# madmann91/bvh

Measured on AMD Instinct MI355X. Metric: Mrays/s closest-hit (1M-tri scene), higher is better.
Workload: dtype f32; 1 GPU; soup_1m: 1,000,000-triangle random soup (M3), worst-case incoherent; robust traversal, DefaultBuilder with thread pool (mini-trees) Quality::High built on the GPU (the reference's default configuration is thread pool + High); rays reordered for coherence inside the timed pass (library default for this tree size); tris=1000000, nodes=1866439, ray_batches=4, parallelism=single GPU, launched_by=single process

## Files before the change

### bvh_amd/csrc/ray_key.h

```cpp
#pragma once

namespace bvh_amd {

namespace {

__device__ inline float rcp_fast(float x) { return __builtin_amdgcn_rcpf(x); }
__device__ inline double rcp_fast(double x) { return 1.0 / x; }
template <typename T>
__device__ inline uint32_t ray_key(const T (&r)[8], T lx, T ly, T lz, T sx, T sy, T sz, uint32_t cells, int hilbert_bits, int class_bits, T class_scale) {
    const T q[3] = { (r[0] - lx) * sx, (r[1] - ly) * sy, (r[2] - lz) * sz };
    uint32_t code = 0;
    uint32_t cell[3];
#pragma unroll
    for (int k = 0; k < 3; ++k) {
        T v = q[k];
        v = v > T(0) ? v : T(0);
        cell[k] = v >= T(cells - 1) ? cells - 1 : static_cast<uint32_t>(v);
    }
    if (hilbert_bits > 0) {
        uint32_t X[3] = { cell[2], cell[1], cell[0] };
        const uint32_t M = 1u << (hilbert_bits - 1);
        for (uint32_t Q = M; Q > 1; Q >>= 1) {
            const uint32_t P = Q - 1;
#pragma unroll
            for (int a = 0; a < 3; ++a) {
                if (X[a] & Q) X[0] ^= P;
                else { const uint32_t t = (X[0] ^ X[a]) & P; X[0] ^= t; X[a] ^= t; }
            }
        }
        X[1] ^= X[0]; X[2] ^= X[1];
        uint32_t t = 0;
        for (uint32_t Q = M; Q > 1; Q >>= 1) if (X[2] & Q) t ^= Q - 1;
        X[0] ^= t; X[1] ^= t; X[2] ^= t;
        cell[2] = X[0]; cell[1] = X[1]; cell[0] = X[2];
    }
#pragma unroll
    for (int k = 0; k < 3; ++k) {
        const uint32_t c = cell[k];
        uint32_t s = (c & 1u) | ((c & 2u) << 2) | ((c & 4u) << 4) | ((c & 8u) << 6) | ((c & 16u) << 8) | ((c & 32u) << 10) | ((c & 64u) << 12) | ((c & 128u) << 14);
        code |= s << k;
    }
    const uint32_t oct = (Num<T>::sign(r[3]) ? 1u : 0u) | (Num<T>::sign(r[4]) ? 2u : 0u) | (Num<T>::sign(r[5]) ? 4u : 0u);
    if (class_bits > 0) {
        const T l[3] = { lx, ly, lz }, sc[3] = { sx, sy, sz };
        T t0 = r[6], t1 = r[7], d2 = T(0), diag2 = T(0);
#pragma unroll
        for (int k = 0; k < 3; ++k) {
            const T ext = sc[k] > T(0) ? T(cells) * rcp_fast(sc[k]) : T(0);
            const T inv = rcp_fast(r[3 + k]);
            const T a = (l[k] - r[k]) * inv, b = (l[k] + ext - r[k]) * inv;
            const T lo_t = a < b ? a : b, hi_t = a < b ? b : a;
            t0 = lo_t > t0 ? lo_t : t0; t1 = hi_t < t1 ? hi_t : t1;
            d2 += r[3 + k] * r[3 + k]; diag2 += ext * ext;
        }
        const uint32_t top = (1u << class_bits) - 1u;
        uint32_t cls = 0;
        const T len = t1 > t0 ? t1 - t0 : T(0);
        if (class_bits == 1) cls = len * len * d2 * class_scale * class_scale >= diag2 && diag2 > T(0) ? 1u : 0u;
        else {
            const T rel = diag2 > T(0) ? len * Num<T>::sqrt_(d2) / Num<T>::sqrt_(diag2) * class_scale : T(0);
            cls = rel >= T(top) ? top : rel > T(0) ? static_cast<uint32_t>(rel) : 0u;
        }
        cls = top - cls;
        const int code_bits = 3 * (hilbert_bits > 0 ? hilbert_bits : 31 - __clz(cells));
        const uint32_t high = code >> (code_bits - 3), low = (code & ((1u << (code_bits - 3)) - 1u)) >> class_bits;
        code = (((high << class_bits) | cls) << (code_bits - 3 - class_bits)) | low;
    }
    return (code << 3) | oct;
}

}

}
```

### bvh_amd/csrc/trace_body.inc

```
#ifndef BVH_TRACE_COOP
#define BVH_TRACE_COOP false
#endif
    constexpr int kDepth = kLdsDepth;
    constexpr int kSpill = 64 - kDepth;
    __shared__ uint32_t lds_stack[kDepth * kBlock];
    uint32_t spill[kSpill];
    const int tid = threadIdx.x;
    const int lane = tid & (kWave - 1);
    const uint64_t lanes_below = (uint64_t{1} << lane) - 1;

    bool have = false, done = false, drained = false, nan_ray = false;
    uint32_t part = a.parts > 1 ? blockIdx.x % a.parts : 0, parts_left = a.parts;
    unsigned long long ray_id = 0;
    T org[3], dir[3], inv[3], aux[3];
    T tmin = 0, tmax = 0;
    uint32_t oct[3] = {0, 0, 0};
    uint32_t top = 0, sp = 0;
    uint32_t hit_prim = BVH_AMD_INVALID;
    T hit_t = 0, hit_u = 0, hit_v = 0;
    unsigned long long n_pairs = 0, n_tests = 0, n_leaves = 0;
#if defined(BVH_AMD_DEVELOPER) && defined(__HIPCC__)
    unsigned long long wt_begin = 0, wt_last_refill = 0, wt_rays = 0, wt_refill_ticks = 0, wt_refills = 0;
    if (a.wave_times) wt_begin = __builtin_amdgcn_s_memrealtime();
#endif

    auto deep_slot = [&](uint32_t i) { return a.deep + (size_t{blockIdx.x} * kBlock + tid) * a.deep_cap + i; };
    auto push = [&](uint32_t v) {
        if (sp < kDepth) lds_stack[sp * kBlock + tid] = v;
        else if (!Deep) spill[min(sp - kDepth, static_cast<uint32_t>(kSpill - 1))] = v;
        else if (sp < kDepth + kSpill) spill[sp - kDepth] = v;
        else *deep_slot(min(sp - (kDepth + kSpill), a.deep_cap - 1)) = v;
        ++sp;
    };
    auto pop = [&]() -> uint32_t {
        --sp;
        uint32_t v = lds_word(&lds_stack[min(sp, static_cast<uint32_t>(kDepth - 1)) * kBlock + tid]);
        if (sp >= kDepth) {
            if (!Deep) v = spill[min(sp - kDepth, static_cast<uint32_t>(kSpill - 1))];
            else if (sp < kDepth + kSpill) v = spill[sp - kDepth];
            else v = *deep_slot(min(sp - (kDepth + kSpill), a.deep_cap - 1));
        }
        return v;
    };

    for (;;) {
        const uint64_t idle = __ballot(!have);
        const int n_idle = __popcll(idle);
        if (!drained && (n_idle >= a.refill_threshold || n_idle == kWave)) {
#if defined(BVH_AMD_DEVELOPER) && defined(__HIPCC__)
            unsigned long long wt_t0 = 0;
            if (a.wave_times) wt_t0 = __builtin_amdgcn_s_memrealtime();
#endif
            unsigned long long base = 0, part_end = a.n;
            if (a.one_shot) {
                base = (static_cast<unsigned long long>(blockIdx.x) * (kBlock / kWave) + (tid >> 6)) * kWave;
                drained = true;
            } else {
                if (lane == 0) base = atomicAdd(a.work + part * kTicketStride, static_cast<unsigned long long>(n_idle));
                base = __shfl(base, 0) + part * a.part_size;
                part_end = min(a.n, (part + 1ull) * a.part_size);
                if (base + n_idle >= part_end) {
                    part = part + 1 == a.parts ? 0 : part + 1;
                    if (--parts_left == 0) drained = true;
                } else if (a.stagger && part_end - (base + n_idle) < static_cast<unsigned long long>(a.stagger) * ((blockIdx.x * 8u) / gridDim.x)) {
                    drained = true;
                }
            }
            if (!have) {
                const unsigned long long ticket = base + __popcll(idle & lanes_below);
                if (ticket < part_end) {
                    const bool once = (a.stream_hints & 1u) != 0;
                    const unsigned long long my = a.order ? (once ? load_word_nt(a.order + ticket) : a.order[ticket]) : ticket;
                    T r[8];
                    if (D == 3) { if (once) load_ray_nt(a.rays + 8 * my, r); else load_ray(a.rays + 8 * my, r); }
                    else {
                        T q[6];
                        load_ray2(a.rays + 6 * my, q);
                        r[0] = q[0]; r[1] = q[1]; r[2] = T(0); r[3] = q[2]; r[4] = q[3]; r[5] = T(0); r[6] = q[4]; r[7] = q[5];
                    }
#pragma unroll
                    for (int k = 0; k < D; ++k) { org[k] = r[k]; dir[k] = r[3 + k]; }
                    ray_constants<T, Robust, D>(org, dir, inv, aux, oct);
                    tmin = r[6]; tmax = r[7];
                    nan_ray = !(tmin == tmin) || !(tmax == tmax);
                    ray_id = my;
                    have = true; done = false;
                    sp = 0;
                    top = a.root_index;
                    hit_prim = BVH_AMD_INVALID; hit_t = tmax; hit_u = 0; hit_v = 0;
                }
            }
#if defined(BVH_AMD_DEVELOPER) && defined(__HIPCC__)
            if (a.wave_times) {
                asm volatile("s_waitcnt vmcnt(0)" ::: "memory");
                wt_last_refill = __builtin_amdgcn_s_memrealtime(); wt_rays += __popcll(__ballot(have)) - (kWave - n_idle);
                wt_refill_ticks += wt_last_refill - wt_t0; ++wt_refills;
            }
#endif
        }
        if (__ballot(have) == 0) {
            if (drained) break;
            continue;
        }

        for (;;) {
            const bool inner = have && !done && (top & kCountMask) == 0;
            const uint64_t inner_mask = __ballot(inner);
            if (!inner_mask) break;
            const int parked = __popcll(__ballot(have && !done && (top & kCountMask) != 0));
            if (parked >= a.leaf_threshold) break;
            T lb[6], rb[6];
            uint32_t li = 0, ri = 0;
            if constexpr (BVH_TRACE_COOP) coop_load_pair(a.pairs, a.pair_bytes, inner ? (top >> (kCountBits + 1)) : 0xFFFFFFFFu, lane, lb, rb, li, ri);
            if (inner) {
                if constexpr (!BVH_TRACE_COOP) load_pair(a.pairs + (top >> (kCountBits + 1)), lb, rb, li, ri);
                if (Stats) ++n_pairs;
                T l0, l1, r0, r1;
                slab_pair<T, Robust, D>(lb, rb, org, inv, aux, oct, tmin, tmax, l0, l1, r0, r1);
                const bool hl = !nan_ray && l0 <= l1, hr = !nan_ray && r0 <= r1;
                if (hl) {
                    uint32_t near_i = li;
                    if (hr) {
                        uint32_t far_i = ri;
                        if (!Any && l0 > r0) { near_i = ri; far_i = li; }
                        push(far_i);
                    }
                    top = near_i;
                } else if (hr) {
                    top = ri;
                } else if (sp == 0) {
                    done = true;
                } else {
                    top = pop();
                }
            }
        }

        if (have && !done && (top & kCountMask) != 0) {
            const uint32_t first = top >> kCountBits, count = top & kCountMask;
            if (Stats) ++n_leaves;
            for (uint32_t i = first; i < first + count; ++i) {
                if (Stats) ++n_tests;
                if (Leaf == LEAF_TRIANGLE) {
// ... 66 lines not shown
```

### bvh_amd/csrc/trace_device.h

```cpp
#pragma once

#if defined(__HIPCC__)
#define BVH_AMD_KEEP_APART(v) asm volatile("" : "+v"(v))
#else
#define BVH_AMD_KEEP_APART(v) asm volatile("" : "+r"(v))
#endif

namespace bvh_amd {

namespace {

constexpr int kBlock = 256;
constexpr int kLdsDepth = 20;
constexpr int kRefillThreshold = 36;
constexpr int kRefillThresholdSmall = 20;
constexpr int kLeafThreshold = 12;
constexpr int kCoopRefillAny = 20, kCoopLeafAny = 20;
constexpr int kCoopRefillHeavy = 12, kCoopLeafHeavy = 12;


template <typename T> struct Num;
template <> struct Num<float> {
    static constexpr float kMax = 3.402823466e+38f, kEps = 1.1920928955078125e-07f;
    __device__ static bool finite(float x) { return (__float_as_uint(x) & 0x7F800000u) != 0x7F800000u; }
// ... 17 lines not shown
    __device__ static double sqrt_(double x) { return __builtin_sqrt(x); }
    __device__ static double abs_(double x) { return __builtin_fabs(x); }
    __device__ static double copysign_(double a, double b) { return __builtin_copysign(a, b); }
    __device__ static double max_num(double a, double b) { return __builtin_fmax(a, b); }
    __device__ static double min_num(double a, double b) { return __builtin_fmin(a, b); }
};

template <typename T> __device__ inline T pick_min(T a, T b) { return a < b ? a : b; }
template <typename T> __device__ inline T pick_max(T a, T b) { return a > b ? a : b; }

template <typename T> __device__ inline T dot3(T a0, T a1, T a2, T b0, T b1, T b2) {
    return ((T(0) + a0 * b0) + a1 * b1) + a2 * b2;
}
__device__ inline uint32_t lds_word(const uint32_t* shared) {
#if defined(__HIP_DEVICE_COMPILE__)
    typedef __attribute__((address_space(3))) const volatile uint32_t LdsWord;
    return *(LdsWord*)shared;
#else
    return *shared;
#endif
}

template <typename T> __device__ inline T dot2(T a0, T a1, T b0, T b1) { return (T(0) + a0 * b0) + a1 * b1; }

template <typename T, bool Robust, int D>
__device__ inline void ray_constants(const T (&org)[3], const T (&dir)[3], T (&inv)[3], T (&aux)[3], uint32_t (&oct)[3]) {
#pragma unroll
    for (int k = 0; k < D; ++k) {
        const T d = dir[k];
        const T iv = Robust ? T(1) / d : (Num<T>::abs_(d) <= Num<T>::kEps ? Num<T>::copysign_(Num<T>::kMax, d) : T(1) / d);
        inv[k] = iv;
        aux[k] = Robust ? (Num<T>::finite(iv) ? Num<T>::bump2(iv) : iv) : (-iv) * org[k];
        oct[k] = Num<T>::sign(d) ? 1u : 0u;
    }
}

template <typename T, bool Robust, int D>
__device__ inline void slab_pair(const T (&lb)[6], const T (&rb)[6], const T (&org)[3], const T (&inv)[3], const T (&aux)[3], const uint32_t (&oct)[3],
                                 T tmin, T tmax, T& l0, T& l1, T& r0, T& r1) {
    l0 = tmin; l1 = tmax; r0 = tmin; r1 = tmax;
#pragma unroll
    for (int k = 0; k < D; ++k) {
        const T ln = oct[k] ? lb[2 * k + 1] : lb[2 * k], lf = oct[k] ? lb[2 * k] : lb[2 * k + 1];
        const T rn = oct[k] ? rb[2 * k + 1] : rb[2 * k], rf = oct[k] ? rb[2 * k] : rb[2 * k + 1];
        T la, lz, ra, rz;
        if (Robust) {
            la = (ln - org[k]) * inv[k]; lz = (lf - org[k]) * aux[k];
            ra = (rn - org[k]) * inv[k]; rz = (rf - org[k]) * aux[k];
        } else {
            la = Num<T>::fma_(ln, inv[k], aux[k]); lz = Num<T>::fma_(lf, inv[k], aux[k]);
            ra = Num<T>::fma_(rn, inv[k], aux[k]); rz = Num<T>::fma_(rf, inv[k], aux[k]);
        }
        l0 = Num<T>::max_num(la, l0); l1 = Num<T>::min_num(lz, l1);
        r0 = Num<T>::max_num(ra, r0); r1 = Num<T>::min_num(rz, r1);
    }
}

constexpr uint32_t kTicketStride = 16;

template <typename T>
struct TraceArgs {
    const PairNode<T>* pairs;
    const T* prims;
    const T* rays;
    typename HitOf<T>::Type* hits;
    unsigned long long n;
    unsigned long long* work;
    unsigned long long part_size;
    uint32_t parts;
    bvh_amd_counters* counters;
    const uint32_t* order;
    uint32_t* deep;
    uint32_t deep_cap;
    uint32_t root_index;
    int refill_threshold;
    int leaf_threshold;
    uint32_t coop;
    uint32_t prim_stride;
    uint32_t stream_hints;
    uint32_t stagger;
    uint32_t one_shot;
    unsigned long long* wave_times;
    uint32_t pair_bytes = 0;
};

__device__ inline void load_pair(const PairNode<float>* p, float (&lb)[6], float (&rb)[6], uint32_t& li, uint32_t& ri) {
    const float4* q = reinterpret_cast<const float4*>(p);
    float4 a = q[0], b = q[1], c = q[2];
    uint2 d = reinterpret_cast<const uint2*>(p)[6];
    lb[0] = a.x; lb[1] = a.y; lb[2] = a.z; lb[3] = a.w; lb[4] = b.x; lb[5] = b.y;
    rb[0] = b.z; rb[1] = b.w; rb[2] = c.x; rb[3] = c.y; rb[4] = c.z; rb[5] = c.w;
    li = d.x; ri = d.y;
}
__device__ inline void load_pair(const PairNode<double>* p, double (&lb)[6], double (&rb)[6], uint32_t& li, uint32_t& ri) {
    const double2* q = reinterpret_cast<const double2*>(p);
#pragma unroll
    for (int i = 0; i < 3; ++i) { double2 v = q[i]; lb[2 * i] = v.x; lb[2 * i + 1] = v.y; }
#pragma unroll
    for (int i = 0; i < 3; ++i) { double2 v = q[3 + i]; rb[2 * i] = v.x; rb[2 * i + 1] = v.y; }
    uint2 d = reinterpret_cast<const uint2*>(p)[12];
    li = d.x; ri = d.y;
}

#if defined(__HIPCC__)
template <int CTRL> __device__ inline uint32_t quad_perm(uint32_t v) {
    return static_cast<uint32_t>(__builtin_amdgcn_mov_dpp(static_cast<int>(v), CTRL, 0xF, 0xF, true));
}
template <bool ByTwo> __device__ inline void quad_exchange4(uint32_t (&a)[4], uint32_t (&b)[4]) {
    const uint64_t lower = ByTwo ? 0x3333333333333333ull : 0x5555555555555555ull;
    uint32_t n0, n1, n2, n3;
    if (ByTwo)
        asm("s_nop 1\n\ts_mov_b64 vcc, %12\n\t"
            "v_cndmask_b32_dpp %0, %4, %8, vcc quad_perm:[2,3,0,1] row_mask:0xf bank_mask:0xf\n\t"
            "v_cndmask_b32_dpp %1, %5, %9, vcc quad_perm:[2,3,0,1] row_mask:0xf bank_mask:0xf\n\t"
            "v_cndmask_b32_dpp %2, %6, %10, vcc quad_perm:[2,3,0,1] row_mask:0xf bank_mask:0xf\n\t"
            "v_cndmask_b32_dpp %3, %7, %11, vcc quad_perm:[2,3,0,1] row_mask:0xf bank_mask:0xf\n\t"
            "s_not_b64 vcc, vcc\n\t"
            "v_cndmask_b32_dpp %4, %8, %4, vcc quad_perm:[2,3,0,1] row_mask:0xf bank_mask:0xf\n\t"
            "v_cndmask_b32_dpp %5, %9, %5, vcc quad_perm:[2,3,0,1] row_mask:0xf bank_mask:0xf\n\t"
            "v_cndmask_b32_dpp %6, %10, %6, vcc quad_perm:[2,3,0,1] row_mask:0xf bank_mask:0xf\n\t"
            "v_cndmask_b32_dpp %7, %11, %7, vcc quad_perm:[2,3,0,1] row_mask:0xf bank_mask:0xf"
            : "=&v"(n0), "=&v"(n1), "=&v"(n2), "=&v"(n3), "+v"(b[0]), "+v"(b[1]), "+v"(b[2]), "+v"(b[3])
            : "v"(a[0]), "v"(a[1]), "v"(a[2]), "v"(a[3]), "s"(lower) : "vcc", "scc");
    else
        asm("s_nop 1\n\ts_mov_b64 vcc, %12\n\t"
            "v_cndmask_b32_dpp %0, %4, %8, vcc quad_perm:[1,0,3,2] row_mask:0xf bank_mask:0xf\n\t"
            "v_cndmask_b32_dpp %1, %5, %9, vcc quad_perm:[1,0,3,2] row_mask:0xf bank_mask:0xf\n\t"
            "v_cndmask_b32_dpp %2, %6, %10, vcc quad_perm:[1,0,3,2] row_mask:0xf bank_mask:0xf\n\t"
            "v_cndmask_b32_dpp %3, %7, %11, vcc quad_perm:[1,0,3,2] row_mask:0xf bank_mask:0xf\n\t"
            "s_not_b64 vcc, vcc\n\t"
            "v_cndmask_b32_dpp %4, %8, %4, vcc quad_perm:[1,0,3,2] row_mask:0xf bank_mask:0xf\n\t"
            "v_cndmask_b32_dpp %5, %9, %5, vcc quad_perm:[1,0,3,2] row_mask:0xf bank_mask:0xf\n\t"
            "v_cndmask_b32_dpp %6, %10, %6, vcc quad_perm:[1,0,3,2] row_mask:0xf bank_mask:0xf\n\t"
            "v_cndmask_b32_dpp %7, %11, %7, vcc quad_perm:[1,0,3,2] row_mask:0xf bank_mask:0xf"
            : "=&v"(n0), "=&v"(n1), "=&v"(n2), "=&v"(n3), "+v"(b[0]), "+v"(b[1]), "+v"(b[2]), "+v"(b[3])
            : "v"(a[0]), "v"(a[1]), "v"(a[2]), "v"(a[3]), "s"(lower) : "vcc", "scc");
    a[0] = n0; a[1] = n1; a[2] = n2; a[3] = n3;
}
#elif defined(BVH_HOST_WAVE64)
template <int CTRL> inline uint32_t quad_perm(uint32_t v) {
    const int l = static_cast<int>(threadIdx.x) & 63;
    return wave_read(v, (l & ~3) | ((CTRL >> (2 * (l & 3))) & 3), true);
}
template <bool ByTwo> inline void quad_exchange4(uint32_t (&a)[4], uint32_t (&b)[4]) {
    const int l = static_cast<int>(threadIdx.x) & 63, bit = ByTwo ? 2 : 1, partner = l ^ bit;
    const bool lower = (l & bit) == 0;
    for (int i = 0; i < 4; ++i) {
        const uint32_t pa = wave_read(a[i], partner, true), pb = wave_read(b[i], partner, true);
        const uint32_t na = lower ? a[i] : pb, nb = lower ? pa : b[i];
        a[i] = na; b[i] = nb;
    }
}
#endif
constexpr uint32_t kNoRecordAt = 0xFFFFFFFFu << 6;
#if defined(__HIPCC__)
using PairRsrc = __amdgpu_buffer_rsrc_t;
__device__ inline PairRsrc pair_rsrc(const void* base, uint32_t bytes) {
    return __builtin_amdgcn_make_buffer_rsrc(const_cast<void*>(base), 0, static_cast<int>(bytes), 0x00020000);
}
__device__ inline uint4 load_chunk(PairRsrc r, uint32_t at) {
    const auto v = __builtin_amdgcn_raw_buffer_load_b128(r, static_cast<int>(at), 0, 0);
    return uint4{v[0], v[1], v[2], v[3]};
}
#elif defined(BVH_HOST_WAVE64)
struct PairRsrc { const char* base; };
inline PairRsrc pair_rsrc(const void* base, uint32_t) { return PairRsrc{static_cast<const char*>(base)}; }
// ... 130 lines not shown
```

### bvh_amd/csrc/traverse.hip

```cpp

#include "common.h"
#include "trace_device.h"
#include "ray_key.h"

#include <algorithm>
#include <cstdlib>
#include <mutex>
#include <thread>
#include <type_traits>
#include <vector>

namespace bvh_amd {

namespace {

thread_local const char* g_last_kernel = "";
thread_local bool g_last_reordered = false;
thread_local int g_last_query_launches = 0;
thread_local int g_last_plan[4] = {0, 0, 0, 0};

struct KernelTimer {
    static constexpr size_t kRing = 256;
    bool on = false;
    size_t count = 0;
    std::pair<hipEvent_t, hipEvent_t> ring[kRing] = {};
    hipEvent_t begin[kRing] = {};
    bool begin_armed = false;
};
KernelTimer& kernel_timer() { static thread_local KernelTimer t; return t; }

template <typename T, bool Any, bool Robust, int Leaf, bool Stats, int D = 3, bool Deep = false>
__global__ void __launch_bounds__(kBlock) trace_kernel(TraceArgs<T> a) {
#include "trace_body.inc"
}

template <typename T, bool Any, bool Robust, int Leaf, bool Stats>
__global__ void __launch_bounds__(kBlock, 8) trace_kernel_coop(TraceArgs<T> a) {
    constexpr int D = 3;
    constexpr bool Deep = false;
#undef BVH_TRACE_COOP
#define BVH_TRACE_COOP true
#include "trace_body.inc"
#undef BVH_TRACE_COOP
}

template <typename T, bool Any, bool Robust, int Leaf, bool Stats, int D>
__global__ void __launch_bounds__(kBlock, sizeof(T) == 4 ? 8 : 4) trace_kernel_coop_nd(TraceArgs<T> a) {
    constexpr bool Deep = false;
#undef BVH_TRACE_COOP
#define BVH_TRACE_COOP true
#include "trace_body.inc"
#undef BVH_TRACE_COOP
}

template <typename T, bool Any, bool Robust, int Leaf>
__global__ void __launch_bounds__(kBlock) trace_kernel_plan_search(TraceArgs<T> a) {
    constexpr int D = 3;
    constexpr bool Deep = false, Stats = false;
#include "trace_body.inc"
}
template <typename T, bool Any, bool Robust, int Leaf>
__global__ void __launch_bounds__(kBlock, 8) trace_kernel_coop_plan_search(TraceArgs<T> a) {
    constexpr int D = 3;
    constexpr bool Deep = false, Stats = false;
#undef BVH_TRACE_COOP
#define BVH_TRACE_COOP true
#include "trace_body.inc"
#undef BVH_TRACE_COOP
}

#if defined(BVH_AMD_DEVELOPER)
__global__ void __launch_bounds__(256) k_check_order(const uint32_t* order, uint32_t n, uint32_t* bad) {
    const uint32_t i = blockIdx.x * 256 + threadIdx.x;
    if (i < n && order[i] >= n) {
        const uint32_t k = atomicAdd(&bad[0], 1u);
        if (k < 3) { bad[1 + 2 * k] = i; bad[2 + 2 * k] = order[i]; }
    }
}
#endif

template <typename T>
__global__ void __launch_bounds__(1024) ray_keys_kernel(const T* rays, uint32_t n, T lx, T ly, T lz, T sx, T sy, T sz, uint32_t* keys, uint32_t cells,
                                                        int hilbert_bits, int class_bits, T class_scale, uint32_t* hist, uint32_t tiles) {
    __shared__ uint32_t h[256];
    if (threadIdx.x < 256) h[threadIdx.x] = 0;
    __syncthreads();
    const uint32_t base = blockIdx.x * uint32_t(kRadixTileU32);
#pragma unroll
    for (int s0 = 0; s0 < kRadixTileU32 / 1024; ++s0) {
        const uint32_t i = base + uint32_t(s0) * 1024u + threadIdx.x;
        if (i < n) {
            T r[8];
            load_ray_nt(rays + 8ull * i, r);
            const uint32_t key = ray_key<T>(r, lx, ly, lz, sx, sy, sz, cells, hilbert_bits, class_bits, class_scale);
            keys[i] = key;
            atomicAdd(&h[key & 0xFFu], 1u);
        }
    }
    __syncthreads();
    if (threadIdx.x < 256) hist[size_t{threadIdx.x} * tiles + blockIdx.x] = h[threadIdx.x];
}

__global__ void __launch_bounds__(256) ray_entry_keys_kernel(const float* rays, uint32_t n, const PairNode<float>* pairs, uint32_t root_index, int depth,
                                                             uint32_t* keys) {
    const uint32_t i = blockIdx.x * 256 + threadIdx.x;
    if (i >= n) return;
    float r[8];
    load_ray(rays + 8ull * i, r);
    const float inv[3] = { 1.0f / r[3], 1.0f / r[4], 1.0f / r[5] };
    uint32_t cur = root_index, path = 0;
    int level = 0;
    for (; level < depth && (cur & kCountMask) == 0; ++level) {
        float lb[6], rb[6];
        uint32_t li, ri;
        load_pair(pairs + (cur >> (kCountBits + 1)), lb, rb, li, ri);
        float t0[2] = { r[6], r[6] }, t1[2] = { r[7], r[7] };
#pragma unroll
        for (int k = 0; k < 3; ++k) {
            const float a0 = (lb[2 * k] - r[k]) * inv[k], a1 = (lb[2 * k + 1] - r[k]) * inv[k];
            const float b0 = (rb[2 * k] - r[k]) * inv[k], b1 = (rb[2 * k + 1] - r[k]) * inv[k];
            t0[0] = fmaxf(t0[0], fminf(a0, a1)); t1[0] = fminf(t1[0], fmaxf(a0, a1));
            t0[1] = fmaxf(t0[1], fminf(b0, b1)); t1[1] = fminf(t1[1], fmaxf(b0, b1));
        }
        const bool hl = t0[0] <= t1[0], hr = t0[1] <= t1[1];
        if (!hl && !hr) break;
        const bool right = hl && hr ? t0[1] < t0[0] : hr;
        path = (path << 1) | (right ? 1u : 0u);
        cur = right ? ri : li;
    }
    path <<= (depth - level);
    const uint32_t oct = (Num<float>::sign(r[3]) ? 1u : 0u) | (Num<float>::sign(r[4]) ? 2u : 0u) | (Num<float>::sign(r[5]) ? 4u : 0u);
    keys[i] = (path << 3) | oct;
}

template <typename H>
__global__ void __launch_bounds__(256) original_ids_kernel(H* hits, size_t n, const uint32_t* prim_ids, uint32_t prim_count) {
    const size_t i = blockIdx.x * size_t{256} + threadIdx.x;
    if (i >= n) return;
    const uint32_t p = hits[i].prim;
    if (p < prim_count) hits[i].prim = prim_ids[p];
}

thread_local int t_refill = -1, t_leaf = -1, t_coop = -1, t_parts = -1;
struct Experiments { int grid_blocks = -1, stream_hints = -1, tri_stride = -1, key_curve = -1, key_bits = -1, wave_times = -1, one_shot = -1,
                     key_class_bits = -1, key_class_scale = -1, stagger = -1; };
constexpr int kKeyClassBits = 0, kKeyClassScalePercent = 500;
constexpr uint32_t kStaggerHeavy = 100000, kStaggerLight = 50000, kStaggerDouble = 20000;
thread_local bool g_last_classes = false;
thread_local float g_search_ns[5] = {0, 0, 0, 0, 0};
thread_local int g_search_count[5] = {0, 0, 0, 0, 0};
thread_local unsigned g_search_dropped = 0;
thread_local Experiments t_exp;
#if defined(BVH_AMD_DEVELOPER)
constexpr size_t kWaveTimeWords = 6, kWaveTimeWaves = 8 * 256 * (kBlock / kWave) * 2;
thread_local unsigned long long* t_wave_times = nullptr;
thread_local size_t t_wave_times_waves = 0;
#endif
thread_local std::pair<hipEvent_t, hipEvent_t>* t_calibration = nullptr;

int coop_fetch_forced() {
    static const int knob = BVH_DEV_INT("BVH_AMD_COOP", -1);
    return t_coop >= 0 ? (t_coop != 0) : knob < 0 ? -1 : (knob != 0);
}

struct Grid { int blocks = 0; };

template <typename K>
int persistent_grid(K kernel, int device, Grid& g) {
    int per_cu = 0, cus = 0;
    BVH_HIP_TRY(hipOccupancyMaxActiveBlocksPerMultiprocessor(&per_cu, kernel, kBlock, 0), BVH_AMD_ERR_HIP);
    BVH_HIP_TRY(hipDeviceGetAttribute(&cus, hipDeviceAttributeMultiprocessorCount, device), BVH_AMD_ERR_HIP);
    if (per_cu < 1) per_cu = 1;
    if (per_cu > 8) per_cu = 8;
    g.blocks = per_cu * cus;
    return BVH_AMD_OK;
}

template <typename T, bool Any, bool Robust, int Leaf, bool Stats, int D, bool Deep, bool Coop = false>
int launch_variant_d(const BvhImpl<T>& b, const TraceArgs<T>& args, hipStream_t stream, const char* name) {
    static thread_local int cached_blocks[16] = {0};
    void (*kernel)(TraceArgs<T>) = nullptr;
    constexpr bool CoopNd = Coop && !(std::is_same_v<T, float> && D == 3);
    if constexpr (CoopNd) kernel = trace_kernel_coop_nd<T, Any, Robust, Leaf, Stats, D>;
    else if constexpr (Coop) kernel = trace_kernel_coop<T, Any, Robust, Leaf, Stats>;
    else kernel = trace_kernel<T, Any, Robust, Leaf, Stats, D, Deep>;
    if constexpr (std::is_same_v<T, float> && D == 3 && !Deep && !Stats) {
        if (t_calibration) {
            if constexpr (Coop) kernel = trace_kernel_coop_plan_search<T, Any, Robust, Leaf>;
            else kernel = trace_kernel_plan_search<T, Any, Robust, Leaf>;
        }
    }
    int& blocks = cached_blocks[b.device & 15];
    if (blocks == 0) {
        Grid g;
        int rc = persistent_grid(kernel, b.device, g);
        if (rc) return rc;
        blocks = g.blocks;
    }
    unsigned long long need = (args.n + kBlock - 1) / kBlock;
    int grid = static_cast<int>(need < static_cast<unsigned long long>(blocks) ? need : blocks);
    if (args.one_shot) grid = static_cast<int>(need);
    else if constexpr (!Coop && std::is_same_v<T, float>) {
        int cus = blocks / 7 > 0 ? blocks / 7 : 1;
        (void)hipDeviceGetAttribute(&cus, hipDeviceAttributeMultiprocessorCount, b.device);
        const int cap = 6 * cus;
        if (grid > cap) grid = cap;
    }
    static const int grid_env = BVH_DEV_INT("BVH_AMD_GRID_BLOCKS", 0);
    if (!args.one_shot) {
        if (grid_env > 0 && grid > grid_env) grid = grid_env;
        if (t_exp.grid_blocks > 0 && grid > t_exp.grid_blocks) grid = t_exp.grid_blocks;
    }
    if (grid < 1) grid = 1;
    (void)name;
    static const std::string head = std::string(CoopNd ? "trace_kernel_coop_nd<" : Coop ? "trace_kernel_coop<" : "trace_kernel<") + (std::is_same_v<T, float> ? "float" : "double") + ", " +
                                    (Any ? "true" : "false") + ", " + (Robust ? "true" : "false") + ", " + std::to_string(Leaf) + ", " + (Stats ? "true" : "false");
    static const std::string symbol = CoopNd ? head + ", " + std::to_string(D) + ">" : Coop ? head + ">" : head + ", " + std::to_string(D) + ", " + (Deep ? "true" : "false") + ">";
    g_last_kernel = symbol.c_str();
    KernelTimer& timer = kernel_timer();
    hipEvent_t stop = nullptr;
    if (timer.on) {
        std::pair<hipEvent_t, hipEvent_t>& ev = timer.ring[timer.count % KernelTimer::kRing];
        if (!timer.begin_armed && timer.begin[timer.count % KernelTimer::kRing]) {
            (void)hipEventDestroy(timer.begin[timer.count % KernelTimer::kRing]);
            timer.begin[timer.count % KernelTimer::kRing] = nullptr;
        }
        timer.begin_armed = false;
        if (!ev.first) {
            BVH_HIP_TRY(hipEventCreate(&ev.first), BVH_AMD_ERR_HIP);
            BVH_HIP_TRY(hipEventCreate(&ev.second), BVH_AMD_ERR_HIP);
        }
        BVH_HIP_TRY(hipEventRecord(ev.first, stream), BVH_AMD_ERR_HIP);
        stop = ev.second;
        ++timer.count;
    }
    if (t_calibration) (void)hipEventRecord(t_calibration->first, stream);
#if defined(BVH_AMD_DEVELOPER)
    TraceArgs<T> timed_args = args;
    if (t_exp.wave_times > 0 && size_t(grid) * (kBlock / kWave) <= kWaveTimeWaves) {
        if (!t_wave_times) BVH_HIP_TRY(hipMalloc(&t_wave_times, kWaveTimeWaves * kWaveTimeWords * sizeof(unsigned long long)), BVH_AMD_ERR_HIP);
        t_wave_times_waves = size_t(grid) * (kBlock / kWave);
        BVH_HIP_TRY(hipMemsetAsync(t_wave_times, 0, t_wave_times_waves * kWaveTimeWords * sizeof(unsigned long long), stream), BVH_AMD_ERR_HIP);
        timed_args.wave_times = t_wave_times;
    }
    hipLaunchKernelGGL(kernel, dim3(grid), dim3(kBlock), 0, stream, timed_args);
#else
    hipLaunchKernelGGL(kernel, dim3(grid), dim3(kBlock), 0, stream, args);
#endif
    BVH_HIP_TRY(hipGetLastError(), BVH_AMD_ERR_HIP);
    if (t_calibration) (void)hipEventRecord(t_calibration->second, stream);
    if (stop) BVH_HIP_TRY(hipEventRecord(stop, stream), BVH_AMD_ERR_HIP);
    return BVH_AMD_OK;
}

template <typename T, bool Any, bool Robust, int Leaf, bool Stats, int D>
int launch_variant(const BvhImpl<T>& b, const TraceArgs<T>& args, hipStream_t stream, const char* name) {
    if (args.deep) return launch_variant_d<T, Any, Robust, Leaf, Stats, D, true>(b, args, stream, name);
    if (args.coop && b.pair_count < (size_t{1} << (std::is_same_v<T, float> ? 26 : 25))) return launch_variant_d<T, Any, Robust, Leaf, Stats, D, false, true>(b, args, stream, name);
    return launch_variant_d<T, Any, Robust, Leaf, Stats, D, false>(b, args, stream, name);
}

#define BVH_VARIANT(T, ANY, ROB, LEAF, STATS) \
    launch_variant<T, ANY, ROB, LEAF, STATS, D>(b, args, stream, D == 3 ? "trace_kernel<" #T "," #ANY "," #ROB "," #LEAF "," #STATS ">" \
                                                                        : "trace_kernel<" #T "," #ANY "," #ROB "," #LEAF "," #STATS ",2>")

template <typename T, int Leaf, int D = 3>
int dispatch(const BvhImpl<T>& b, const TraceArgs<T>& args, unsigned flags, bool stats, hipStream_t stream) {
    const bool any = flags & BVH_AMD_RAY_ANY_HIT, rob = flags & BVH_AMD_RAY_ROBUST;
    if (stats) {
        if (any) return rob ? BVH_VARIANT(T, true, true, Leaf, true) : BVH_VARIANT(T, true, false, Leaf, true);
        return rob ? BVH_VARIANT(T, false, true, Leaf, true) : BVH_VARIANT(T, false, false, Leaf, true);
    }
    if (any) return rob ? BVH_VARIANT(T, true, true, Leaf, false) : BVH_VARIANT(T, true, false, Leaf, false);
    return rob ? BVH_VARIANT(T, false, true, Leaf, false) : BVH_VARIANT(T, false, false, Leaf, false);
}

}

void last_launch_plan(int out[4]) { for (int k = 0; k < 4; ++k) out[k] = g_last_plan[k]; }
void set_tuning(int refill, int leaf, int coop, int parts) { t_refill = refill; t_leaf = leaf; t_coop = coop; t_parts = parts; }
int set_experiment(const char* name, int value) {
    const std::string k = name ? name : "";
    if (k == "grid_blocks") t_exp.grid_blocks = value;
    else if (k == "stream_hints") t_exp.stream_hints = value;
    else if (k == "tri_stride") t_exp.tri_stride = value;
    else if (k == "key_curve") t_exp.key_curve = value;
    else if (k == "key_bits") t_exp.key_bits = value;
    else if (k == "step_events") set_step_events(value);
    else if (k == "one_shot") t_exp.one_shot = value;
    else if (k == "stagger") t_exp.stagger = value;
    else if (k == "key_class_bits") t_exp.key_class_bits = value;
    else if (k == "key_class_scale") t_exp.key_class_scale = value;
    else if (k == "wave_times") {
#if defined(BVH_AMD_DEVELOPER)
        t_exp.wave_times = value;
#else
        return fail(BVH_AMD_ERR_ARG, "bvh_amd_experiment: 'wave_times' exists in the developer library only (python -m bvh_amd.build --developer)");
#endif
    }
    else if (k == "reset") { t_exp = Experiments{}; set_step_events(-1); }
    else return fail(BVH_AMD_ERR_ARG, "bvh_amd_experiment: unknown knob '" + k + "'");
    return BVH_AMD_OK;
}
int wave_times(unsigned long long* out, size_t capacity_waves, size_t* n_waves) {
#if defined(BVH_AMD_DEVELOPER)
    if (n_waves) *n_waves = t_wave_times_waves;
    if (!out || !t_wave_times) return BVH_AMD_OK;
    BVH_HIP_TRY(hipDeviceSynchronize(), BVH_AMD_ERR_HIP);
    BVH_HIP_TRY(hipMemcpy(out, t_wave_times, std::min(capacity_waves, t_wave_times_waves) * kWaveTimeWords * sizeof(unsigned long long), hipMemcpyDeviceToHost), BVH_AMD_ERR_HIP);
    return BVH_AMD_OK;
#else
    (void)out; (void)capacity_waves;
    if (n_waves) *n_waves = 0;
    return fail(BVH_AMD_ERR_ARG, "bvh_amd_wave_times: developer library only");
#endif
}
void last_plan_search(float ns_per_ray[5], int measurements[5], unsigned* dropped) {
    for (int c = 0; c < 5; ++c) { if (ns_per_ray) ns_per_ray[c] = g_search_ns[c]; if (measurements) measurements[c] = g_search_count[c]; }
    if (dropped) *dropped = g_search_dropped;
}
const char* last_kernel_name() { return g_last_kernel; }
bool last_launch_reordered() { return g_last_reordered; }
int last_query_launches() { return g_last_query_launches; }
void set_last_query_launches(int launches) { g_last_query_launches = launches; }

void kernel_timing(bool on) {
    KernelTimer& t = kernel_timer();
    t.on = on;
    t.count = 0;
}

int kernel_times(float* ms_out, size_t capacity, size_t* count_out) {
    KernelTimer& t = kernel_timer();
    const size_t have = std::min<size_t>(t.count, KernelTimer::kRing), n = std::min(have, capacity);
    for (size_t i = 0; i < n; ++i) {
        const std::pair<hipEvent_t, hipEvent_t>& ev = t.ring[(t.count - n + i) % KernelTimer::kRing];
        BVH_HIP_TRY(hipEventSynchronize(ev.second), BVH_AMD_ERR_HIP);
        BVH_HIP_TRY(hipEventElapsedTime(&ms_out[i], ev.first, ev.second), BVH_AMD_ERR_HIP);
    }
    if (count_out) *count_out = n;
    return BVH_AMD_OK;
}

int reorder_times(float* ms_out, size_t capacity, size_t* count_out) {
    KernelTimer& t = kernel_timer();
    const size_t have = std::min<size_t>(t.count, KernelTimer::kRing), n = std::min(have, capacity);
    for (size_t i = 0; i < n; ++i) {
        const size_t k = (t.count - n + i) % KernelTimer::kRing;
        ms_out[i] = 0.0f;
        if (!t.begin[k]) continue;
        BVH_HIP_TRY(hipEventSynchronize(t.ring[k].first), BVH_AMD_ERR_HIP);
        BVH_HIP_TRY(hipEventElapsedTime(&ms_out[i], t.begin[k], t.ring[k].first), BVH_AMD_ERR_HIP);
    }
    if (count_out) *count_out = n;
    return BVH_AMD_OK;
}

template <typename T>
static int to_original_ids(const BvhImpl<T>& b, typename HitOf<T>::Type* d_hits, size_t n, hipStream_t stream) {
    if (!b.d_prim_ids) return fail(BVH_AMD_ERR_ARG, "intersect_rays: BVH has no device prim ids");
    hipLaunchKernelGGL(original_ids_kernel<typename HitOf<T>::Type>, dim3(static_cast<unsigned>((n + 255) / 256)), dim3(256), 0, stream, d_hits, n,
                       b.d_prim_ids, static_cast<uint32_t>(b.prim_count));
    BVH_HIP_TRY(hipGetLastError(), BVH_AMD_ERR_HIP);
    return BVH_AMD_OK;
}

constexpr float kReorderMinVisits = 100.0f;

struct Plan { bool reorder; bool coop; int refill, leaf; bool classes = false; };

template <typename T>
static int launch_planned(const BvhImpl<T>& b, int leaf_kind, const T* d_prims, const T* d_rays, size_t n, unsigned flags,
                          typename HitOf<T>::Type* d_hits, bvh_amd_counters* d_counters, hipStream_t stream, const Plan* plan)
{
    if (n == 0) return BVH_AMD_OK;
// ... 29 lines not shown
        if (ev) timer.begin_armed = hipEventRecord(ev, stream) == hipSuccess;
    }
    TraceArgs<T> args{};
    args.pairs = b.d_pairs; args.prims = d_prims; args.rays = d_rays; args.hits = d_hits;
    args.pair_bytes = static_cast<uint32_t>(std::min<size_t>(b.pair_count * sizeof(PairNode<T>), 0xFFFFFFFFu));
    args.n = n; args.work = work; args.counters = d_counters; args.root_index = b.root_index;
    args.order = nullptr;
    args.prim_stride = leaf_kind == LEAF_TRIANGLE ? (t_exp.tri_stride > 0 ? static_cast<uint32_t>(t_exp.tri_stride) : 12u) : 4u;
    args.stream_hints = 0;
    args.one_shot = (t_exp.one_shot >= 0 ? t_exp.one_shot > 0 : n <= (size_t{1} << 18)) && !d_counters ? 1u : 0u;
    static const int parts_env = BVH_DEV_INT("BVH_AMD_PARTS", 0);
    args.parts = t_parts > 0 ? std::min(t_parts, 256) : parts_env > 0 ? std::min(parts_env, 256) : n < 65536 ? 1 : 8;
    args.part_size = ((n + args.parts - 1) / args.parts + 63) / 64 * 64;
    args.deep = nullptr; args.deep_cap = 0;
    StreamScope scope(stream);
    void* deep_mem = nullptr;
    void* sort_mem = nullptr;
    ScratchTag deep_tag, sort_tag;
    auto release = [&](int rc) {
        (void)hipEventRecord(slot_event, stream);
        { std::lock_guard<std::mutex> lock(b.work_mutex); b.work_busy[slot] = false; }
        if (deep_mem) scratch_free(deep_mem, deep_tag);
        if (sort_mem) scratch_free(sort_mem, sort_tag);
        return rc;
    };
    if (d_counters) {
        const hipError_t e = hipMemsetAsync(d_counters, 0, sizeof(bvh_amd_counters), stream);
        if (e != hipSuccess) return release(fail(BVH_AMD_ERR_HIP, std::string("intersect_rays: hipMemsetAsync: ") + hipGetErrorString(e)));
    }
    {
        int rc = tree_depth<T>(b, stream);
        if (rc) return release(rc);
        const int max_depth = b.max_depth.load();
        if (max_depth > 64) {
            int cus = 0;
            if (hipDeviceGetAttribute(&cus, hipDeviceAttributeMultiprocessorCount, b.device) != hipSuccess) return release(fail(BVH_AMD_ERR_HIP, "intersect_rays: hipDeviceGetAttribute"));
            const size_t lanes = size_t{8} * cus * kBlock;
            const size_t cap = static_cast<size_t>(max_depth - 64 + 1);
            if (lanes * cap > (size_t{1} << 32))
                return release(fail(BVH_AMD_ERR_UNSUPPORTED, "intersect_rays: the tree is too deep for the traversal stack (" + std::to_string(max_depth) + " levels)"));
            const hipError_t e = scratch_alloc(&deep_mem, lanes * cap * sizeof(uint32_t), &deep_tag);
            if (e != hipSuccess) { deep_mem = nullptr; return release(fail(BVH_AMD_ERR_HIP, std::string("intersect_rays: stack spill buffer: ") + hipGetErrorString(e))); }
            args.deep = static_cast<uint32_t*>(deep_mem); args.deep_cap = static_cast<uint32_t>(cap);
            args.one_shot = 0;
        }
    }
    static const int refill_env = BVH_DEV_INT("BVH_AMD_REFILL", 0);
    static const int leaf_env = BVH_DEV_INT("BVH_AMD_LEAF", 0);
    const bool beyond_l2 = b.pair_count * sizeof(PairNode<T>) > (size_t{32} << 20);
    const bool heavy = beyond_l2 && b.expected_visits.load() >= kReorderMinVisits;
    const bool any_hit = (flags & BVH_AMD_RAY_ANY_HIT) != 0;
    const int forced = coop_fetch_forced();
    const bool coop_capable = true;
    if (plan) {
        args.coop = coop_capable && plan->coop ? 1u : 0u;
        args.refill_threshold = plan->refill; args.leaf_threshold = plan->leaf;
    } else {
        args.coop = (coop_capable && (forced >= 0 ? forced != 0 : (any_hit || (heavy && n >= (size_t{1} << 21))))) ? 1u : 0u;
        const int refill_lane = n <= (size_t{1} << 21) && std::is_same_v<T, float> ? kRefillThresholdSmall : kRefillThreshold;
        const int refill_default = !args.coop ? refill_lane : any_hit ? kCoopRefillAny : heavy ? kCoopRefillHeavy : kCoopRefillAny;
        const int leaf_default = !args.coop ? kLeafThreshold : any_hit ? kCoopLeafAny : heavy ? kCoopLeafHeavy : kCoopLeafAny;
        args.refill_threshold = t_refill > 0 ? t_refill : refill_env > 0 ? refill_env : refill_default;
        args.leaf_threshold = t_leaf > 0 ? t_leaf : leaf_env > 0 ? leaf_env : leaf_default;
    }
    auto zero_tickets = [&]() -> int {
        const hipError_t e = hipMemsetAsync(work, 0, size_t{args.parts} * kTicketStride * sizeof(unsigned long long), stream);
        return e == hipSuccess ? BVH_AMD_OK : fail(BVH_AMD_ERR_HIP, std::string("intersect_rays: hipMemsetAsync: ") + hipGetErrorString(e));
    };
    if (b.dim == 2) {
        if (leaf_kind != LEAF_SPHERE) return release(fail(BVH_AMD_ERR_ARG, "intersect_rays: a 2D BVH traces circles (Sphere<T, 2>) only"));
        if (const int rc0 = zero_tickets()) return release(rc0);
        int rc2 = dispatch<T, LEAF_SPHERE, 2>(b, args, flags, d_counters != nullptr, stream);
        if (rc2 == BVH_AMD_OK && (flags & BVH_AMD_RAY_ORIGINAL_IDS)) rc2 = to_original_ids<T>(b, d_hits, n, stream);
        return release(rc2);
    }
    const bool reorder = (flags & BVH_AMD_RAY_SORTED) ? n > 4096
                       : (flags & BVH_AMD_RAY_UNSORTED) ? false
                       : plan ? plan->reorder && n > 4096
                       : n >= (size_t{1} << 20) && beyond_l2 && b.expected_visits.load() >= kReorderMinVisits;
    g_last_reordered = reorder && n < (size_t{1} << 31);
    args.stream_hints = t_exp.stream_hints >= 0 ? static_cast<uint32_t>(t_exp.stream_hints) : g_last_reordered ? 1u : 0u;
    args.parts = t_parts > 0 ? std::min(t_parts, 256) : parts_env > 0 ? std::min(parts_env, 256) : n < 65536 ? 1 : g_last_reordered ? 8 : 32;
    args.part_size = ((n + args.parts - 1) / args.parts + 63) / 64 * 64;
    if (const int rc0 = zero_tickets()) return release(rc0);
    if (g_last_reordered) {
        const uint32_t n32 = static_cast<uint32_t>(n);
        const size_t words = 4 * n + radix_sort_hist_words(n32, 1);
        hipError_t e = scratch_alloc(&sort_mem, words * sizeof(uint32_t), &sort_tag);
        if (e != hipSuccess) {
            sort_mem = nullptr;
            (void)hipGetLastError();
            if (flags & BVH_AMD_RAY_SORTED) return release(fail(BVH_AMD_ERR_HIP, std::string("intersect_rays: no scratch for BVH_AMD_RAY_SORTED: ") + hipGetErrorString(e)));
            g_last_reordered = false;
        }
    }
    if (g_last_reordered) {
        const uint32_t n32 = static_cast<uint32_t>(n);
        uint32_t *keys = static_cast<uint32_t*>(sort_mem), *vals = keys + n, *kt = vals + n, *vt = kt + n, *hist = vt + n;
        T lo[3], sc[3];
        if (const int rc0 = b.wait_refit()) return release(rc0);
        for (int k = 0; k < 3; ++k) {
            const T ext = b.root_bounds[2 * k + 1] - b.root_bounds[2 * k];
            lo[k] = b.root_bounds[2 * k];
            sc[k] = ext > T(0) ? T(64) / ext : T(0);
        }
        static const int entry_depth = std::min(29, BVH_DEV_INT("BVH_AMD_RAY_KEY_DEPTH", 0));
        int key_bits = 21;
        bool entry_keys = false, first_hist_done = false;
        if constexpr (std::is_same_v<T, float>) entry_keys = entry_depth > 0 && b.dim == 3;
        if constexpr (std::is_same_v<T, float>) {
            if (entry_keys) {
                hipLaunchKernelGGL(ray_entry_keys_kernel, dim3((n32 + 255) / 256), dim3(256), 0, stream, d_rays, n32, args.pairs, args.root_index, entry_depth, keys);
                key_bits = entry_depth + 3;
            }
        }
        if (!entry_keys) {
            static const int cell_bits_env = std::max(1, std::min(8, BVH_DEV_INT("BVH_AMD_RAY_KEY_BITS", 7)));
            const int cell_bits = t_exp.key_bits > 0 ? std::min(8, t_exp.key_bits) : cell_bits_env;
            const T rescale = static_cast<T>(1u << cell_bits) / T(64);
            const int class_bits = cell_bits < 3 ? 0 : t_exp.key_class_bits >= 0 ? std::min(3, t_exp.key_class_bits) : (plan && plan->classes) ? 1 : kKeyClassBits;
            g_last_classes = class_bits > 0;
            const T class_scale = static_cast<T>(t_exp.key_class_scale > 0 ? t_exp.key_class_scale : kKeyClassScalePercent) / T(100);
            const uint32_t tiles = (n32 + kRadixTileU32 - 1) / kRadixTileU32;
            hipLaunchKernelGGL(ray_keys_kernel<T>, dim3(tiles), dim3(1024), 0, stream, d_rays, n32, lo[0], lo[1], lo[2], sc[0] * rescale, sc[1] * rescale,
                               sc[2] * rescale, keys, 1u << cell_bits, t_exp.key_curve == 0 ? 0 : cell_bits,
                               class_bits, class_scale, hist, tiles);
            first_hist_done = true;
            key_bits = 3 * cell_bits + 3;
        }
        uint32_t* order = nullptr;
        int rc = radix_sort_pairs<uint32_t>(keys, vals, kt, vt, n32, 1, key_bits, stream, hist, true, false, &order, first_hist_done);
        if (rc) return release(rc);
        args.order = order;
#if defined(BVH_AMD_DEVELOPER)
        if (getenv("BVH_AMD_CHECK_ORDER")) {
            uint32_t* d_bad = nullptr;
            if (hipMalloc(&d_bad, 8 * sizeof(uint32_t)) == hipSuccess) {
                for (int round = 0; round < 2; ++round) {
                    (void)hipMemsetAsync(d_bad, 0, 8 * sizeof(uint32_t), stream);
                    hipLaunchKernelGGL(k_check_order, dim3((n32 + 255) / 256), dim3(256), 0, stream, order, n32, d_bad);
                    uint32_t bad[8] = {};
                    (void)hipMemcpyAsync(bad, d_bad, sizeof(bad), hipMemcpyDeviceToHost, stream);
                    (void)hipStreamSynchronize(stream);
                    if (bad[0]) {
                        std::vector<uint32_t> host(n32);
                        (void)hipMemcpy(host.data(), order, size_t{n32} * 4, hipMemcpyDeviceToHost);
                        uint32_t host_bad = 0;
                        for (uint32_t v : host) host_bad += v >= n32 ? 1u : 0u;
                        fprintf(stderr, "[check order] look %d: the copy engine sees %u bad entries\n", round, host_bad);
                    }
                    if (bad[0]) fprintf(stderr, "[check order] look %d: %u of %u entries are not ray indices; first at %u = 0x%x, %u = 0x%x, %u = 0x%x (sort_mem %p, order %p)\n", round, bad[0], n32,
                                        bad[1], bad[2], bad[3], bad[4], bad[5], bad[6], sort_mem, static_cast<void*>(order));
                }
                (void)hipFree(d_bad);
            }
        }
#endif
    }
    {
        const size_t dflt = std::is_same_v<T, double> ? std::min<size_t>(n / 64, kStaggerDouble)
                                                      : std::min<size_t>(n / 16, heavy ? kStaggerHeavy : kStaggerLight);
        const size_t whole = t_exp.stagger > 0 ? static_cast<size_t>(t_exp.stagger) : t_exp.stagger == 0 ? 0 : dflt;
        args.stagger = whole ? std::max<uint32_t>(1u, static_cast<uint32_t>(whole / args.parts)) : 0u;
    }
    g_last_plan[0] = g_last_reordered ? (g_last_classes ? 2 : 1) : 0; g_last_plan[1] = static_cast<int>(args.coop); g_last_plan[2] = args.refill_threshold; g_last_plan[3] = args.leaf_threshold;
    int rc = leaf_kind == LEAF_TRIANGLE ? dispatch<T, LEAF_TRIANGLE>(b, args, flags, d_counters != nullptr, stream)
                                        : dispatch<T, LEAF_SPHERE>(b, args, flags, d_counters != nullptr, stream);
    if (rc == BVH_AMD_OK && (flags & BVH_AMD_RAY_ORIGINAL_IDS)) rc = to_original_ids<T>(b, d_hits, n, stream);
    return release(rc);
}


constexpr float kSortNsPerRay = 0.031f;

static uint32_t pack_plan(const Plan& p) { return 1u | (p.reorder ? 2u : 0u) | (p.coop ? 4u : 0u) | (p.classes ? 8u : 0u) | (uint32_t(p.refill) << 8) | (uint32_t(p.leaf) << 16); }
static Plan unpack_plan(uint32_t w) { return Plan{(w & 2u) != 0, (w & 4u) != 0, int((w >> 8) & 0xFFu), int((w >> 16) & 0xFFu), (w & 8u) != 0}; }

template <typename T>
int launch_traverse(const BvhImpl<T>& b, int leaf_kind, const T* d_prims, const T* d_rays, size_t n, unsigned flags,
                    typename HitOf<T>::Type* d_hits, bvh_amd_counters* d_counters, hipStream_t stream)
{
    static const bool calibrate_on = !(getenv("BVH_AMD_CALIBRATE") && atoi(getenv("BVH_AMD_CALIBRATE")) == 0);
    const bool any_hit = (flags & BVH_AMD_RAY_ANY_HIT) != 0;
    const int kind = any_hit ? 1 : 0;
    const bool free_choice = !(flags & (BVH_AMD_RAY_SORTED | BVH_AMD_RAY_UNSORTED)) && coop_fetch_forced() < 0 && t_refill <= 0 && t_leaf <= 0 &&
                             !BVH_DEV_STR("BVH_AMD_REFILL") && !BVH_DEV_STR("BVH_AMD_LEAF");
    const bool candidate = calibrate_on && free_choice && b.dim == 3 && n >= (size_t{1} << 20) && n < (size_t{1} << 31) &&
                           b.pair_count * sizeof(PairNode<T>) > (size_t{32} << 20);
    if (!candidate) return launch_planned<T>(b, leaf_kind, d_prims, d_rays, n, flags, d_hits, d_counters, stream, nullptr);
    if (b.node_count && b.d_pairs) {
        const int rc = tree_depth<T>(b, stream);
        if (rc) return rc;
    }
    if (const uint32_t cached = b.launch_plan[kind].load()) {
        const Plan plan = unpack_plan(cached);
        return launch_planned<T>(b, leaf_kind, d_prims, d_rays, n, flags, d_hits, d_counters, stream, &plan);
    }
    constexpr int kCand = BvhImpl<T>::PlanSearch::kCandidates;
    const int n_cand = any_hit ? 4 : 5;
    const Plan candidates[kCand] = {
        {false, false, kRefillThreshold, kLeafThreshold},
        {false, true, any_hit ? kCoopRefillAny : kCoopRefillHeavy, any_hit ? kCoopLeafAny : kCoopLeafHeavy},
        any_hit ? Plan{false, true, kCoopRefillHeavy, kCoopLeafHeavy} : Plan{true, false, kRefillThreshold, kLeafThreshold},
        {true, true, any_hit ? kCoopRefillAny : kCoopRefillHeavy, any_hit ? kCoopLeafAny : kCoopLeafHeavy},
        {true, true, kCoopRefillHeavy, kCoopLeafHeavy, true},
    };
    const bool heavy = b.expected_visits.load() >= kReorderMinVisits;
    const bool fits_infinity_cache = b.pair_count * sizeof(PairNode<T>) <= (size_t{256} << 20);
    const int predicted = any_hit ? (heavy ? 3 : 1) : (heavy ? (fits_infinity_cache ? 4 : 3) : 0);
    int order[kCand], n_order = 0;
    {
        auto push = [&](int c) { for (int k = 0; k < n_order; ++k) if (order[k] == c) return; order[n_order++] = c; };
        push(predicted);
        for (int c = 0; c < n_cand; ++c) if (candidates[c].reorder != candidates[predicted].reorder && candidates[c].coop == candidates[predicted].coop && !candidates[c].classes) push(c);
        for (int c = 0; c < n_cand; ++c)
            if (c != predicted && candidates[c].reorder && candidates[predicted].reorder && candidates[c].coop == candidates[predicted].coop) push(c);
// ... 132 lines not shown
```

Measured before the change: 2433 Mrays/s.

## Add tail class to ray keys and align ticket ranges to key-prefix boundaries

Result: faster. 2556 Mrays/s (median of 6 runs) (+5.1%).

```diff
diff --git a/bvh_amd/csrc/ray_key.h b/bvh_amd/csrc/ray_key.h
--- a/bvh_amd/csrc/ray_key.h
+++ b/bvh_amd/csrc/ray_key.h
@@ -4,10 +4,15 @@
 
 namespace {
 
+#if defined(__HIPCC__)
 __device__ inline float rcp_fast(float x) { return __builtin_amdgcn_rcpf(x); }
+#else
+inline float rcp_fast(float x) { return 1.0f / x; }
+#endif
 __device__ inline double rcp_fast(double x) { return 1.0 / x; }
 template <typename T>
-__device__ inline uint32_t ray_key(const T (&r)[8], T lx, T ly, T lz, T sx, T sy, T sz, uint32_t cells, int hilbert_bits, int class_bits, T class_scale) {
+__device__ inline uint32_t ray_key(const T (&r)[8], T lx, T ly, T lz, T sx, T sy, T sz, uint32_t cells, int hilbert_bits, int class_bits, T class_scale,
+                                   T tail_frac = T(-1)) {
     const T q[3] = { (r[0] - lx) * sx, (r[1] - ly) * sy, (r[2] - lz) * sz };
     uint32_t code = 0;
     uint32_t cell[3];
@@ -55,16 +60,23 @@
         }
         const uint32_t top = (1u << class_bits) - 1u;
         uint32_t cls = 0;
+        int field_bits = class_bits;
         const T len = t1 > t0 ? t1 - t0 : T(0);
-        if (class_bits == 1) cls = len * len * d2 * class_scale * class_scale >= diag2 && diag2 > T(0) ? 1u : 0u;
-        else {
+        if (class_bits == 1) {
+            const T len2 = len * len * d2;
+            cls = len2 * class_scale * class_scale >= diag2 && diag2 > T(0) ? 0u : 1u;
+            if (tail_frac >= T(0)) {
+                if (cls != 0u && !(len2 > tail_frac * tail_frac * diag2)) cls = 2u;
+                field_bits = 2;
+            }
+        } else {
             const T rel = diag2 > T(0) ? len * Num<T>::sqrt_(d2) / Num<T>::sqrt_(diag2) * class_scale : T(0);
             cls = rel >= T(top) ? top : rel > T(0) ? static_cast<uint32_t>(rel) : 0u;
+            cls = top - cls;
         }
-        cls = top - cls;
         const int code_bits = 3 * (hilbert_bits > 0 ? hilbert_bits : 31 - __clz(cells));
-        const uint32_t high = code >> (code_bits - 3), low = (code & ((1u << (code_bits - 3)) - 1u)) >> class_bits;
-        code = (((high << class_bits) | cls) << (code_bits - 3 - class_bits)) | low;
+        const uint32_t high = code >> (code_bits - 3), low = (code & ((1u << (code_bits - 3)) - 1u)) >> field_bits;
+        code = (((high << field_bits) | cls) << (code_bits - 3 - field_bits)) | low;
     }
     return (code << 3) | oct;
 }
diff --git a/bvh_amd/csrc/trace_body.inc b/bvh_amd/csrc/trace_body.inc
--- a/bvh_amd/csrc/trace_body.inc
+++ b/bvh_amd/csrc/trace_body.inc
@@ -57,8 +57,10 @@
                 drained = true;
             } else {
                 if (lane == 0) base = atomicAdd(a.work + part * kTicketStride, static_cast<unsigned long long>(n_idle));
-                base = __shfl(base, 0) + part * a.part_size;
+                unsigned long long part_begin = part * a.part_size;
                 part_end = min(a.n, (part + 1ull) * a.part_size);
+                if (a.range_starts) { part_begin = a.range_starts[part]; part_end = a.range_starts[part + 1]; }
+                base = __shfl(base, 0) + part_begin;
                 if (base + n_idle >= part_end) {
                     part = part + 1 == a.parts ? 0 : part + 1;
                     if (--parts_left == 0) drained = true;
diff --git a/bvh_amd/csrc/trace_device.h b/bvh_amd/csrc/trace_device.h
--- a/bvh_amd/csrc/trace_device.h
+++ b/bvh_amd/csrc/trace_device.h
@@ -123,6 +123,7 @@
     uint32_t one_shot;
     unsigned long long* wave_times;
     uint32_t pair_bytes = 0;
+    const uint32_t* range_starts = nullptr;
 };
 
 __device__ inline void load_pair(const PairNode<float>* p, float (&lb)[6], float (&rb)[6], uint32_t& li, uint32_t& ri) {
diff --git a/bvh_amd/csrc/traverse.hip b/bvh_amd/csrc/traverse.hip
--- a/bvh_amd/csrc/traverse.hip
+++ b/bvh_amd/csrc/traverse.hip
@@ -81,7 +81,7 @@
 
 template <typename T>
 __global__ void __launch_bounds__(1024) ray_keys_kernel(const T* rays, uint32_t n, T lx, T ly, T lz, T sx, T sy, T sz, uint32_t* keys, uint32_t cells,
-                                                        int hilbert_bits, int class_bits, T class_scale, uint32_t* hist, uint32_t tiles) {
+                                                        int hilbert_bits, int class_bits, T class_scale, T tail_frac, uint32_t* hist, uint32_t tiles) {
     __shared__ uint32_t h[256];
     if (threadIdx.x < 256) h[threadIdx.x] = 0;
     __syncthreads();
@@ -92,13 +92,28 @@
         if (i < n) {
             T r[8];
             load_ray_nt(rays + 8ull * i, r);
-            const uint32_t key = ray_key<T>(r, lx, ly, lz, sx, sy, sz, cells, hilbert_bits, class_bits, class_scale);
+            const uint32_t key = ray_key<T>(r, lx, ly, lz, sx, sy, sz, cells, hilbert_bits, class_bits, class_scale, tail_frac);
             keys[i] = key;
             atomicAdd(&h[key & 0xFFu], 1u);
         }
     }
     __syncthreads();
     if (threadIdx.x < 256) hist[size_t{threadIdx.x} * tiles + blockIdx.x] = h[threadIdx.x];
+}
+
+__global__ void __launch_bounds__(64) ticket_ranges_kernel(const uint32_t* hist, uint32_t tiles, uint32_t digits_per_prefix, uint32_t n, uint32_t parts,
+                                                           unsigned long long part_size, uint32_t* starts, unsigned long long* work) {
+    const uint32_t p = threadIdx.x;
+    uint32_t begin = n, end = n;
+    if (p < parts) {
+        begin = hist[size_t{p} * digits_per_prefix * tiles];
+        if (p + 1 < parts) end = hist[size_t{p + 1} * digits_per_prefix * tiles];
+    }
+    const uint32_t even = n / parts, len = end - begin;
+    const bool balanced = p >= parts || (begin <= end && end <= n && 4ull * len >= 3ull * even && 4ull * len <= 5ull * even);
+    const bool keep = __ballot(!balanced) == 0;
+    if (p <= parts) starts[p] = keep ? begin : static_cast<uint32_t>(min(static_cast<unsigned long long>(n), p * part_size));
+    if (p < parts) work[p * kTicketStride] = 0;
 }
 
 __global__ void __launch_bounds__(256) ray_entry_keys_kernel(const float* rays, uint32_t n, const PairNode<float>* pairs, uint32_t root_index, int depth,
@@ -143,8 +158,9 @@
 
 thread_local int t_refill = -1, t_leaf = -1, t_coop = -1, t_parts = -1;
 struct Experiments { int grid_blocks = -1, stream_hints = -1, tri_stride = -1, key_curve = -1, key_bits = -1, wave_times = -1, one_shot = -1,
-                     key_class_bits = -1, key_class_scale = -1, stagger = -1; };
+                     key_class_bits = -1, key_class_scale = -1, stagger = -1, key_tail = -1, key_tail_permille = -1, range_align = -1; };
 constexpr int kKeyClassBits = 0, kKeyClassScalePercent = 500;
+constexpr int kKeyTail = 1, kKeyTailPermille = 50, kRangeAlign = 1;
 constexpr uint32_t kStaggerHeavy = 100000, kStaggerLight = 50000, kStaggerDouble = 20000;
 thread_local bool g_last_classes = false;
 thread_local float g_search_ns[5] = {0, 0, 0, 0, 0};
@@ -291,6 +307,9 @@
     else if (k == "stagger") t_exp.stagger = value;
     else if (k == "key_class_bits") t_exp.key_class_bits = value;
     else if (k == "key_class_scale") t_exp.key_class_scale = value;
+    else if (k == "key_tail") t_exp.key_tail = value;
+    else if (k == "key_tail_permille") t_exp.key_tail_permille = value;
+    else if (k == "range_align") t_exp.range_align = value;
     else if (k == "wave_times") {
 #if defined(BVH_AMD_DEVELOPER)
         t_exp.wave_times = value;
@@ -486,10 +505,10 @@
     args.stream_hints = t_exp.stream_hints >= 0 ? static_cast<uint32_t>(t_exp.stream_hints) : g_last_reordered ? 1u : 0u;
     args.parts = t_parts > 0 ? std::min(t_parts, 256) : parts_env > 0 ? std::min(parts_env, 256) : n < 65536 ? 1 : g_last_reordered ? 8 : 32;
     args.part_size = ((n + args.parts - 1) / args.parts + 63) / 64 * 64;
-    if (const int rc0 = zero_tickets()) return release(rc0);
+    constexpr size_t kRangeWords = 64;
     if (g_last_reordered) {
         const uint32_t n32 = static_cast<uint32_t>(n);
-        const size_t words = 4 * n + radix_sort_hist_words(n32, 1);
+        const size_t words = 4 * n + radix_sort_hist_words(n32, 1) + kRangeWords;
         hipError_t e = scratch_alloc(&sort_mem, words * sizeof(uint32_t), &sort_tag);
         if (e != hipSuccess) {
             sort_mem = nullptr;
@@ -498,7 +517,9 @@
             g_last_reordered = false;
         }
     }
-    if (g_last_reordered) {
+    if (!g_last_reordered) {
+        if (const int rc0 = zero_tickets()) return release(rc0);
+    } else {
         const uint32_t n32 = static_cast<uint32_t>(n);
         uint32_t *keys = static_cast<uint32_t*>(sort_mem), *vals = keys + n, *kt = vals + n, *vt = kt + n, *hist = vt + n;
         T lo[3], sc[3];
@@ -525,10 +546,12 @@
             const int class_bits = cell_bits < 3 ? 0 : t_exp.key_class_bits >= 0 ? std::min(3, t_exp.key_class_bits) : (plan && plan->classes) ? 1 : kKeyClassBits;
             g_last_classes = class_bits > 0;
             const T class_scale = static_cast<T>(t_exp.key_class_scale > 0 ? t_exp.key_class_scale : kKeyClassScalePercent) / T(100);
+            const bool tail = class_bits == 1 && cell_bits >= 2 && (t_exp.key_tail >= 0 ? t_exp.key_tail > 0 : kKeyTail > 0);
+            const T tail_frac = tail ? static_cast<T>(t_exp.key_tail_permille >= 0 ? t_exp.key_tail_permille : kKeyTailPermille) / T(1000) : T(-1);
             const uint32_t tiles = (n32 + kRadixTileU32 - 1) / kRadixTileU32;
             hipLaunchKernelGGL(ray_keys_kernel<T>, dim3(tiles), dim3(1024), 0, stream, d_rays, n32, lo[0], lo[1], lo[2], sc[0] * rescale, sc[1] * rescale,
                                sc[2] * rescale, keys, 1u << cell_bits, t_exp.key_curve == 0 ? 0 : cell_bits,
-                               class_bits, class_scale, hist, tiles);
+                               class_bits, class_scale, tail_frac, hist, tiles);
             first_hist_done = true;
             key_bits = 3 * cell_bits + 3;
         }
@@ -536,6 +559,15 @@
         int rc = radix_sort_pairs<uint32_t>(keys, vals, kt, vt, n32, 1, key_bits, stream, hist, true, false, &order, first_hist_done);
         if (rc) return release(rc);
         args.order = order;
+        const int top_digit_bits = key_bits - 8 * ((key_bits + 7) / 8 - 1);
+        const bool align = args.parts == 8 && !args.one_shot && top_digit_bits >= 3 && (t_exp.range_align >= 0 ? t_exp.range_align > 0 : kRangeAlign > 0);
+        if (align) {
+            uint32_t* starts = hist + radix_sort_hist_words(n32, 1);
+            const uint32_t tiles = (n32 + kRadixTileU32 - 1) / kRadixTileU32;
+            hipLaunchKernelGGL(ticket_ranges_kernel, dim3(1), dim3(64), 0, stream, hist, tiles, 1u << (top_digit_bits - 3), n32, args.parts, args.part_size, starts, work);
+            if (const hipError_t e = hipGetLastError(); e != hipSuccess) return release(fail(BVH_AMD_ERR_HIP, std::string("intersect_rays: ticket_ranges_kernel: ") + hipGetErrorString(e)));
+            args.range_starts = starts;
+        } else if (const int rc0 = zero_tickets()) return release(rc0);
 #if defined(BVH_AMD_DEVELOPER)
         if (getenv("BVH_AMD_CHECK_ORDER")) {
             uint32_t* d_bad = nullptr;
```
